# MirceaKitsune/python_raytracer

Measured on AMD Instinct MI355X. Metric: Mrays/s (primary+bounce), higher is better.
Workload: dtype f64; 1 GPU; mods/default 3840x2160 spp8 max_bounces8 (BASELINE config 3/4); width=3840, height=2160, samples=8, primary_rays=62725130, bounce_rays=75192856, partition=(x ^ y) % 1, traversed=True, fast_draws=32, frames_in_flight=1, scene_flow=pre-selected camera chunks (fixture), rng_retraced_rays=0, rng_table=static seeds: draw table + ray table built once before the timed region, reused

## Files before the change

### python_raytracer_amd/csrc/vrt_kernels.hip

```cpp
#include <hip/hip_runtime.h>
#include <stdint.h>
#include <stdio.h>
#include <stdlib.h>
#include <string.h>

#include <atomic>
#include <mutex>
#include <vector>

#include "../../include/vrt.h"
#include "vrt_math.h"

#pragma clang fp contract(off)

#define VRT_WAVE 64
#define VRT_BLOCK 256

static thread_local int g_last_hip_error = 0;
#define HIP_TRY(expr)                                   \
    do {                                                \
        hipError_t e__ = (expr);                        \
        if (e__ != hipSuccess) {                        \
            g_last_hip_error = (int)e__;                \
            return VRT_ERR_HIP;                         \
// ... 8 lines not shown
struct ProfScope {
    hipStream_t s;
    bool on;
    ProfEvent e;
    ProfScope(hipStream_t stream, int kind) : s(stream), on(g_prof_on && ((g_prof_kinds >> kind) & 1u)) {
        if (!on) return;
        e.kind = kind;
        if (hipEventCreate(&e.a) != hipSuccess) { on = false; return; }
        if (hipEventCreate(&e.b) != hipSuccess) { (void)hipEventDestroy(e.a); on = false; return; }
        (void)hipEventRecord(e.a, s);
    }
    ~ProfScope() {
        if (!on) return;
        (void)hipEventRecord(e.b, s);
        std::lock_guard<std::mutex> lock(g_prof_mu);
        g_prof.push_back(e);
    }
};

__host__ __device__ static inline int64_t voxel_offset(int cs, int lx, int ly, int lz) {
    int nb = cs >> 3;
    int brick = (((lx >> 3) * nb) + (ly >> 3)) * nb + (lz >> 3);
    int micro = ((((lx >> 2) & 1) * 2) + ((ly >> 2) & 1)) * 2 + ((lz >> 2) & 1);
    int vox = (((lx & 3) * 4) + (ly & 3)) * 4 + (lz & 3);
    return (int64_t)brick * 512 + micro * 64 + vox;
}

template <class ST>
__host__ __device__ static inline void pixel_setup(const ST& st, int x, int y, double& dir_x, double& dir_y,
                                                   double& detail, int& n) {
    dir_x = -1 + ((double)x / (double)st.width) * 2;
    dir_y = -1 + ((double)y / (double)st.height) * 2;
    detail = 1 - __builtin_fabs(dir_x * dir_y) * st.lod_edge;
    double r = __builtin_rint((double)st.samples * detail);
    n = r > 1 ? (int)r : 1;
}

struct TileGeom {
    const int32_t* pixels;
    int64_t n_px;
    int32_t smax;
};

template <class ST>
__host__ __device__ static inline uint64_t ray_seed(const ST& st, int smax, int x, int y, int s) {
    if (st.seed_nonce == 0) return (uint64_t)((uint32_t)(1 + x) * (uint32_t)(1 + y) * (uint32_t)(1 + s));
    return ((uint64_t)y * (uint64_t)st.width + (uint64_t)x) * (uint64_t)smax + (uint64_t)s + st.seed_nonce;
}

#define VRT_PLAN_MAGIC 0x5652544e414c5032ull
struct PlanHeader {
    uint64_t magic, n_px, n_slots, n_distinct, settings_hash, n_words;
    uint64_t full_frame;
    uint64_t pad;
};
static_assert(sizeof(PlanHeader) == 64, "plan header is 64 bytes");

static uint64_t plan_hash(const vrt_settings* st, int64_t n_px) {
    uint64_t h = 0xcbf29ce484222325ull;
    auto mix = [&](uint64_t v) { h = (h ^ v) * 0x100000001b3ull; };
    union { double d; uint64_t u; } c;
    c.d = st->lod_edge;
    mix((uint64_t)st->width);
    mix((uint64_t)st->height);
    mix((uint64_t)st->samples);
    mix(c.u);
    mix((uint64_t)n_px);
    return h;
}

#define VRT_SCAN_WORDS 1024

__global__ void __launch_bounds__(VRT_BLOCK) plan_mark_kernel(vrt_settings st, TileGeom g, uint32_t* bitmap, PlanHeader* hdr) {
    int64_t p = (int64_t)blockIdx.x * VRT_BLOCK + threadIdx.x;
    if (p >= g.n_px) return;
    int x = g.pixels[2 * p], y = g.pixels[2 * p + 1];
    if ((int64_t)x * st.height + y != p) hdr->full_frame = 0;
    double dx, dy, det;
    int ns;
    pixel_setup(st, x, y, dx, dy, det, ns);
    const uint32_t base = (uint32_t)(1 + x) * (uint32_t)(1 + y);
    for (int s = 0; s < ns; s++) {
        const uint32_t seed = base * (uint32_t)(1 + s);
        const uint32_t bit = 1u << (seed & 31);
        if (!(bitmap[seed >> 5] & bit)) atomicOr(&bitmap[seed >> 5], bit);
    }
}

__global__ void __launch_bounds__(VRT_BLOCK) plan_blocksum_kernel(const uint32_t* bitmap, int64_t n_words,
                                                                   uint32_t* block_sums) {
    __shared__ uint32_t s_sum[VRT_BLOCK / VRT_WAVE];
    int64_t w0 = (int64_t)blockIdx.x * VRT_SCAN_WORDS + threadIdx.x * 4;
    uint32_t c = 0;
    for (int k = 0; k < 4; k++)
        if (w0 + k < n_words) c += __popc(bitmap[w0 + k]);
    for (int o = 32; o > 0; o >>= 1) c += __shfl_down(c, o);
    if ((threadIdx.x & 63) == 0) s_sum[threadIdx.x >> 6] = c;
    __syncthreads();
    if (threadIdx.x == 0) block_sums[blockIdx.x] = s_sum[0] + s_sum[1] + s_sum[2] + s_sum[3];
}

__global__ void __launch_bounds__(VRT_BLOCK) plan_scan_sums_kernel(uint32_t* block_sums, int64_t n_blocks,
                                                                    PlanHeader* hdr) {
    __shared__ uint32_t s_part[VRT_BLOCK];
    __shared__ uint32_t s_carry;
    if (threadIdx.x == 0) s_carry = 0;
    __syncthreads();
    for (int64_t base = 0; base < n_blocks; base += VRT_BLOCK) {
        int64_t i = base + threadIdx.x;
        uint32_t v = i < n_blocks ? block_sums[i] : 0;
        s_part[threadIdx.x] = v;
        __syncthreads();
        for (int o = 1; o < VRT_BLOCK; o <<= 1) {
            uint32_t t = threadIdx.x >= (unsigned)o ? s_part[threadIdx.x - o] : 0;
            __syncthreads();
            s_part[threadIdx.x] += t;
            __syncthreads();
        }
        uint32_t incl = s_part[threadIdx.x];
        uint32_t carry = s_carry;
        if (i < n_blocks) block_sums[i] = carry + incl - v;
        __syncthreads();
        if (threadIdx.x == VRT_BLOCK - 1) s_carry = carry + incl;
        __syncthreads();
    }
    if (threadIdx.x == 0) hdr->n_distinct = s_carry;
}

__global__ void __launch_bounds__(VRT_BLOCK) plan_compact_kernel(const uint32_t* bitmap, int64_t n_words,
                                                                  const uint32_t* block_sums, uint32_t* prefix,
                                                                  uint32_t* seed_list) {
    __shared__ uint32_t s_part[VRT_BLOCK];
    int64_t w0 = (int64_t)blockIdx.x * VRT_SCAN_WORDS + threadIdx.x * 4;
    uint32_t words[4], c = 0;
    for (int k = 0; k < 4; k++) {
        words[k] = (w0 + k < n_words) ? bitmap[w0 + k] : 0;
        c += __popc(words[k]);
    }
    s_part[threadIdx.x] = c;
    __syncthreads();
    for (int o = 1; o < VRT_BLOCK; o <<= 1) {
        uint32_t t = threadIdx.x >= (unsigned)o ? s_part[threadIdx.x - o] : 0;
        __syncthreads();
        s_part[threadIdx.x] += t;
        __syncthreads();
    }
    uint32_t pos = block_sums[blockIdx.x] + s_part[threadIdx.x] - c;
    for (int k = 0; k < 4; k++) {
        if (w0 + k >= n_words) break;
        prefix[w0 + k] = pos;
        uint32_t w = words[k];
        while (w) {
            int b = __ffs(w) - 1;
            w &= w - 1;
            seed_list[pos++] = (uint32_t)((w0 + k) * 32 + b);
        }
    }
}

__global__ void __launch_bounds__(VRT_BLOCK) plan_index_kernel(vrt_settings st, TileGeom g, const uint32_t* bitmap,
                                                                const uint32_t* prefix, uint32_t* ray_seedidx) {
    int64_t i = (int64_t)blockIdx.x * VRT_BLOCK + threadIdx.x;
    if (i >= g.n_px * g.smax) return;
    int64_t p = i / g.smax;
    int s = (int)(i - p * g.smax);
    int x = g.pixels[2 * p], y = g.pixels[2 * p + 1];
    double dx, dy, det;
    int ns;
    pixel_setup(st, x, y, dx, dy, det, ns);
    uint32_t out = 0xffffffffu;
    if (s < ns) {
        const uint32_t seed = (uint32_t)(1 + x) * (uint32_t)(1 + y) * (uint32_t)(1 + s);
        const uint32_t w = bitmap[seed >> 5];
        out = prefix[seed >> 5] + __popc(w & ((1u << (seed & 31)) - 1u));
    }
    ray_seedidx[i] = out;
}

struct MtInit { uint32_t v[624]; };
static constexpr MtInit make_mt_init() {
    MtInit t{};
    t.v[0] = 19650218u;
    for (int i = 1; i < 624; i++) t.v[i] = 1812433253u * (t.v[i - 1] ^ (t.v[i - 1] >> 30)) + (uint32_t)i;
    return t;
}
__constant__ MtInit c_mt_init = make_mt_init();

__device__ __forceinline__ uint32_t mt_temper(uint32_t y) {
    y ^= (y >> 11);
    y ^= (y << 7) & 0x9d2c5680u;
    y ^= (y << 15) & 0xefc60000u;
    y ^= (y >> 18);
    return y;
}
__device__ __forceinline__ uint32_t mt_out(uint32_t sk, uint32_t sk1, uint32_t sk397) {
    uint32_t y = (sk & 0x80000000u) | (sk1 & 0x7fffffffu);
    uint32_t v = sk397 ^ (y >> 1) ^ ((y & 1u) ? 0x9908b0dfu : 0u);
    return mt_temper(v);
}
__device__ __forceinline__ double mt_res53(uint32_t a, uint32_t b) {
    return ((double)(a >> 5) * 67108864.0 + (double)(b >> 6)) * (1.0 / 9007199254740992.0);
}

template <bool PAIR>
__device__ __forceinline__ void mt_seed_draws(uint64_t seed, int D, double* out) {
    const int K = 2 * D;
    const uint32_t key0 = (uint32_t)seed, key1 = (uint32_t)(seed >> 32);
    const uint32_t addA = key0;
    const uint32_t addB = key1 ? key1 + 1u : key0;
    const uint32_t* init = c_mt_init.v;
    uint32_t m = init[0];
    m = (init[1] ^ ((m ^ (m >> 30)) * 1664525u)) + addA;
    const uint32_t first1 = m;
#pragma unroll 2
    for (int i = 2; i < 624; i++) m = (init[i] ^ ((m ^ (m >> 30)) * 1664525u)) + (((i - 1) & 1) ? addB : addA);
    const uint32_t mt1 = (first1 ^ ((m ^ (m >> 30)) * 1664525u)) + ((623 & 1) ? addB : addA);
#define VRT_MT_STEP(p, q, i)                                                            \
    p = (init[i] ^ ((p ^ (p >> 30)) * 1664525u)) + ((((i) - 1) & 1) ? addB : addA);      \
    q = (p ^ ((q ^ (q >> 30)) * 1566083941u)) - (uint32_t)(i);
    uint32_t p = first1, q = mt1;
#pragma unroll 2
    for (int i = 2; i < 397; i++) { VRT_MT_STEP(p, q, i) }
    uint32_t rp = first1, rq = mt1;
    uint32_t s397, s398, s2;
    { VRT_MT_STEP(p, q, 397) }
    s397 = q;
    { VRT_MT_STEP(p, q, 398) }
    s398 = q;
    { VRT_MT_STEP(rp, rq, 2) }
// ... 409 lines not shown
    const uint32_t* list;
    const uint32_t* list_count;
    const double* draws;
    int32_t n_draws, draw_stride;
    int32_t first_draw;
    int32_t per_pixel;
    double lens;
    int32_t t_hit, t_end;
    int32_t max_iters;
    int32_t chunk;
    int32_t brick_lds_off;
    int32_t pool_lds_off;
    int32_t pool_swap_min;
    int32_t pool_refill_min;
    int32_t pool_keep;
    int32_t list_seed;
    union {
        int32_t prefix_draws;
        int32_t slot_stride;
        int32_t max_hits;
    };
    int32_t ct_cells;
    int32_t ct_identity;
    int32_t trav_words;
    int32_t snap_flags;
    int32_t bm_window;
    int32_t wt_on;
    int32_t wt_lds_off;
    int32_t wt_cells[3];
    int32_t wt_min[3];
    int32_t wt_words;
    const uint32_t* wt_table;
    uint32_t* ray_rgba;
    union {
        vrt_ray* rays;
        vrt_hit* hits;
        vrt_cast_ray* out_rays;
    };
    uint64_t* stats;
    uint32_t* retrace_list;
    union {
        uint32_t* retrace_count;
        int32_t* path_counts;
    };
    unsigned long long* pow_global;
    unsigned long long* queue_head;
    const PlanHeader* plan_hdr;
    uint32_t* tile_heads;
    int32_t tile_px_log2;
    int32_t tile_log2;
    int32_t tile_ntx, tile_nty;
    uint32_t retrace_cap;
    uint32_t list_cap;
};
#define VRT_VIEW_WORDS 10
#define VRT_VIEWS_LDS_MAX 96

__device__ __noinline__ int3 snap_generic3(int res, int imx, int imy, int imz, int lx, int ly, int lz) {
    int3 o;
    o.x = (int)__builtin_floor((double)(lx + imx) / (double)res) * res - imx;
    o.y = (int)__builtin_floor((double)(ly + imy) / (double)res) * res - imy;
    o.z = (int)__builtin_floor((double)(lz + imz) / (double)res) * res - imz;
    return o;
}

template <class PT>
__device__ __forceinline__ uint32_t chunk_entry_i(const PT& P, const __attribute__((address_space(3))) uint32_t* ct, int cx, int cy,
                                                  int cz, int d0, int d1, int d2, bool lds, bool identity) {
    if ((unsigned)cx >= (unsigned)d0 || (unsigned)cy >= (unsigned)d1 || (unsigned)cz >= (unsigned)d2) return 0;
    const int i = (cx * d1 + cy) * d2 + cz;
    if (lds) return ct[i];
    if (identity) return (uint32_t)(i + 1) | (1u << 24);
    uint32_t e = P.chunk_table[i];
    asm volatile("" : "+v"(e));
    return e;
}
__device__ __forceinline__ const uint8_t* chunk_base(const MarchParams& P, uint32_t entry) {
    return P.voxels + ((int64_t)((entry & 0xffffffu) - 1u) << (3 * P.cs_shift));
}

__device__ __forceinline__ int trav_cell(bool has_keys, int ccx, int ccy, int ccz, int to0, int to1, int to2, int td0, int td1,
                                         int td2) {
    if (!has_keys) return -1;
    const int cx = ccx - to0;
    const int cy = ccy - to1;
    const int cz = ccz - to2;
    if ((unsigned)cx >= (unsigned)td0 || (unsigned)cy >= (unsigned)td1 || (unsigned)cz >= (unsigned)td2) return -2;
    return (cx * td1 + cy) * td2 + cz;
}

struct PowCache {
    unsigned long long* keys;
    unsigned long long* vals;
    unsigned long long* gkeys;
    unsigned long long* gvals;
};
__device__ __forceinline__ unsigned pow_hash(unsigned long long bits) {
    unsigned h = (unsigned)(bits >> 32) * 0x9e3779b1u + (unsigned)bits * 0x85ebca6bu;
    return h >> 24;
}
#define VRT_PW_PROBES 4
#ifndef VRT_POW_INLINE
#define VRT_POW_INLINE __noinline__
#endif
__device__ VRT_POW_INLINE double pow_miss(unsigned long long* keys, unsigned long long* vals, unsigned long long* gkeys,
                                        unsigned long long* gvals, double x, double y) {
// ... 88 lines not shown
    double d0, d1, d2;
    uint32_t view;
};

__device__ __forceinline__ unsigned long long wave_first_u64(unsigned long long v) {
    const unsigned lo = __builtin_amdgcn_readfirstlane((unsigned)v), hi = __builtin_amdgcn_readfirstlane((unsigned)(v >> 32));
    return ((unsigned long long)hi << 32) | lo;
}

enum { LANE_IDLE = 0, LANE_MARCH = 1, LANE_HIT = 2, LANE_ENDED = 3, LANE_ENDED_BROKE = 4, LANE_ENDED_EXHAUSTED = 5 };
__device__ __forceinline__ int opaque_zero() {
    int z = 0;
    asm volatile("" : "+v"(z));
    return z;
}
enum { COLD_POS = 0, COLD_ROT = 3, COLD_DIST_MIN = 7, COLD_POW_Y, COLD_LOD_BOUNCES, COLD_MAX_LIGHT, COLD_MAX_BOUNCES1,
       COLD_SHUTTER, COLD_CS, COLD_INV_CS, COLD_N };
enum { C_LOOKUP = 0, C_NBR, C_CGET, C_HIT, C_ADV, C_NLOCAL };

typedef __attribute__((address_space(3))) uint32_t lds_u32;
typedef __attribute__((address_space(3))) double lds_f64;
typedef __attribute__((address_space(3))) unsigned long long lds_u64;
typedef __attribute__((address_space(3))) char lds_char;

struct MarchCtx {
    const lds_char* tab;
    int tl[3];
    const lds_u32* ct;
    lds_u32* bm;
    const lds_f64* mats;
    const lds_f64* cold;
    lds_u32* tot;
    PowCache pc;
    __amdgpu_buffer_rsrc_t vox;
    unsigned cs4;
    double cs, inv_cs;
    bool kept_cs;
    bool has_bm, tile;

    int td[3];
    int toc[3], oc[3], dm[3];
    const lds_char* wt;
    int wb[3];
    unsigned cs3;
    const lds_char* vw;
};
#define COLD(i) C.cold[(i) + opaque_zero()]
enum { CF_HAS_BM = 1, CF_CT_LDS = 2, CF_CT_IDENTITY = 4, CF_HAS_KEYS = 8, CF_BM_WINDOW = 16 };

#ifdef VRT_DIAG
enum { DG_PASSES = 0, DG_CYC_REFILL, DG_CYC_MARCH, DG_CYC_HIT, DG_CYC_END, DG_ITERS, DG_MARCH_LANES, DG_HIT_EXEC,
       DG_HIT_LANES, DG_END_EXEC, DG_END_LANES, DG_REFILL_EXEC, DG_REFILL_LANES, DG_WAVE_CYCLES, DG_SNAP_ITERS,
       DG_SNAP_LANES, DG_BRICK_VISITS, DG_SWAPS, DG_SWAP_LANES, DG_EVICT_LANES, DG_CYC_SWAP, DG_VOID_LANES,
#ifdef VRT_DIAG_HIST
       DG_NV1, DG_H1 = DG_NV1 + 8, DG_N = DG_H1 + 8
#else
       DG_N
#endif
};
__device__ unsigned long long g_diag[DG_N];
__device__ unsigned long long g_diag_t[5];
#define DG_ADD(idx_, val_)                                                                                      \
    do {                                                                                                        \
        const unsigned long long v_ = (unsigned long long)(val_);   \
        const unsigned long long e_ = __ballot(1);                                                              \
        if ((int)(threadIdx.x & 63) == __ffsll((long long)e_) - 1) dg.acc[idx_] += v_;                           \
    } while (0)
#define DG_TIME() __builtin_amdgcn_s_memtime()
struct DgLane {
    __attribute__((address_space(3))) unsigned long long* acc;
    unsigned brick;
    unsigned long long bv;
};
#define DG_BRICK()                                                                                                     \
    do {                                                                                                               \
        const unsigned key_ = (((unsigned)(int)__builtin_floor(r.px) >> 3) & 1023u) |                                  \
                              ((((unsigned)(int)__builtin_floor(r.py) >> 3) & 1023u) << 10) |                          \
                              ((((unsigned)(int)__builtin_floor(r.pz) >> 3) & 1023u) << 20);                           \
        dg.bv += key_ != dg.brick ? 1 : 0;                                                                             \
        dg.brick = key_;                                                                                               \
    } while (0)
#else
struct DgLane {};
#define DG_ADD(i, v)
#define DG_BRICK()
#endif
#ifdef VRT_ISA_MARK
#define VRT_MARK(name) asm volatile("; @@" name)
#else
#define VRT_MARK(name)
#endif

__device__ __forceinline__ void floor3_i32(double x, double y, double z, int& fx, int& fy, int& fz) {
    double a, b, c;
    const double magic = 6755399441055744.0;
    asm volatile(
        "s_setreg_imm32_b32 hwreg(HW_REG_MODE, 2, 2), 2\n\t"
        "v_add_f64 %0, %3, %6\n\t"
        "v_add_f64 %1, %4, %6\n\t"
        "v_add_f64 %2, %5, %6\n\t"
        "s_setreg_imm32_b32 hwreg(HW_REG_MODE, 2, 2), 0"
        : "=&v"(a), "=&v"(b), "=&v"(c)
        : "v"(x), "v"(y), "v"(z), "s"(magic));
    fx = __double2loint(a);
    fy = __double2loint(b);
    fz = __double2loint(c);
// ... 1986 lines not shown
        if (tile_ticket(Q, (uint32_t)(ts & 7) * per_head + k, first)) {
            first_ray = first;
            break;
        }
    }
    return ts;
}
#define VRT_POOL_STATE_WORD (13 * 2 * VRT_POOL_SLOTS + 9 * VRT_POOL_SLOTS)
#define VRT_POOL_OFF_WORD (13 * 2 * VRT_POOL_SLOTS + 7 * VRT_POOL_SLOTS)

template <int SPEC, int RESMODE, int PERPIX = 0, bool W = false, bool DEFER = false, bool TILE = false>
__global__ void __launch_bounds__(VRT_BLOCK, VRT_WAVES_PER_SIMD) march_pool_kernel(MarchParams P) {
    static_assert(!TILE || DEFER, "tiled hand-out: the instances for scenes beyond the caches");
    static_assert(!W || (RESMODE != 2 && SPEC == 8), "march_step_w");
    static_assert(!(W && DEFER), "deferred key comparison: the shipped march step");
    __shared__ MarchSharedT<W> S;
    extern __shared__ __align__(16) unsigned char s_dyn[];
    MarchCtx C;
    march_prologue<W>(P, S, s_dyn, C);
    const int wave_in_block = threadIdx.x >> 6;
    const int lane = threadIdx.x & 63;
    lds_u64* const pool = (lds_u64*)(s_dyn + P.pool_lds_off + wave_in_block * VRT_POOL_WAVE_BYTES);
    lds_u32* const pool_state = (lds_u32*)pool + VRT_POOL_STATE_WORD;
    if (lane < VRT_POOL_SLOTS) pool_state[lane] = (uint32_t)LANE_IDLE;
    __syncthreads();

    const int64_t count = P.n;
    const int64_t chunk = P.chunk > 0 ? P.chunk : VRT_CHUNK;
    const int64_t tail_start = count - (int64_t)gridDim.x * (2 * VRT_BLOCK);
    int64_t next = 0, range_end = 0;
    bool more = true;
    bool tiled = false;
    int ts = 0;
    if constexpr (TILE) {
        tiled = P.tile_heads != nullptr && P.plan_hdr->full_frame != 0;
        unsigned xcc = 0;
        xcc = __builtin_amdgcn_s_getreg((3 << 11) | 20);
        ts = (int)(xcc & 7u);
    }

    Ray r;
    ray_clear(r);
    int state = LANE_IDLE;
    SeenList<false> sl = seen_unused();
    LkState lk = lk_unused();
    uint64_t wmin_key = 0;
    DG_LANE(dg);
#ifdef VRT_DIAG
    const unsigned long long dg_t_start = __builtin_amdgcn_s_memrealtime();
    unsigned long long dg_t_empty = 0;
    const unsigned long long dg_start = DG_TIME();
#endif

    auto refill = [&]() {
        unsigned long long idle_mask = __ballot(state == LANE_IDLE);
#ifdef VRT_DIAG
        DG_ADD(DG_REFILL_EXEC, 1);
        DG_ADD(DG_REFILL_LANES, __popcll(idle_mask));
#endif
        while (idle_mask != 0ull && (next < range_end || more)) {
            if (TILE && next >= range_end && tiled) {
                int64_t first = -1;
                ts = tile_take(P, ts, lane, chunk, first);
                if (first < 0) {
                    more = false;
#ifdef VRT_DIAG
                    if (!dg_t_empty) dg_t_empty = __builtin_amdgcn_s_memrealtime();
#endif
                    break;
                }
                next = first;
                range_end = first + chunk;
            } else if (next >= range_end) {
                unsigned long long base = 0;
                if (lane == 0) base = atomicAdd(P.queue_head, (unsigned long long)chunk);
                base = wave_first_u64(base);
                if ((int64_t)base >= count) {
                    more = false;
#ifdef VRT_DIAG
                    if (!dg_t_empty) dg_t_empty = __builtin_amdgcn_s_memrealtime();
#endif
                    break;
                }
                next = (int64_t)base;
                range_end = next + chunk < count ? next + chunk : count;
            }
            const unsigned rank = __builtin_amdgcn_mbcnt_hi((unsigned)(idle_mask >> 32),
                                                            __builtin_amdgcn_mbcnt_lo((unsigned)idle_mask, 0u));
            const int64_t k = next + rank;
            next += __popcll(idle_mask);
            if (state == LANE_IDLE && k < range_end) {
                SeenList<false> none;
                none.n = 0;
                if (take_ray<false, false, PERPIX, W>(P, C, k, r, dg, W ? wmin_key : 0ull, none)) state = LANE_MARCH;
            }
            idle_mask = __ballot(state == LANE_IDLE);
        }
    };
    constexpr bool PASS_COUNTS = W || VRT_PASS_COUNTS;
    int32_t tot[C_NLOCAL];
#pragma unroll
    for (int j = 0; j < C_NLOCAL; j++) tot[j] = 0;
    constexpr bool FUSE_ENDED = (VRT_POOL_FUSE & 1) != 0, FUSE_HIT = (VRT_POOL_FUSE & 2) != 0;
    unsigned pass = 0;
    int stalled = 0;
    for (;; pass++) {
#ifdef VRT_DIAG
        DG_ADD(DG_PASSES, 1);
#endif
        VRT_MARK("pass");
        if (PASS_COUNTS) {
#pragma unroll
            for (int j = 0; j < C_NLOCAL; j++) tot[j] = 0;
        }
        const int sstate = lane < VRT_POOL_SLOTS ? (int)__hip_atomic_load(pool_state + lane, __ATOMIC_RELAXED, __HIP_MEMORY_SCOPE_WAVEFRONT) : -1;
        const bool lane_i = state == LANE_IDLE;
        const unsigned long long l_m = __ballot(state == LANE_MARCH), l_h = __ballot(state == LANE_HIT),
                                 l_e = __ballot(state >= LANE_ENDED), l_i = __ballot(lane_i);
        const unsigned long long s_m = __ballot(sstate == LANE_MARCH), s_h = __ballot(sstate == LANE_HIT),
                                 s_e = __ballot(sstate >= LANE_ENDED), s_f = __ballot(sstate == LANE_IDLE);
        const int n_m = (int)(__popcll(l_m) + __popcll(s_m)), n_h = (int)(__popcll(l_h) + __popcll(s_h)),
                  n_e = (int)(__popcll(l_e) + __popcll(s_e));
        const bool rays_left = next < range_end || more;
        if (stalled > 4096) {
            if (lane == 0) atomicAdd(&S.stats[VRT_S_STALLED], 1ull);
            break;
        }
        const bool evict_ok = rays_left && ((TILE && tiled) ? !(ts & 0x80) : range_end < tail_start);
        const bool can_add = rays_left && (l_i != 0ull || (evict_ok && s_f != 0ull));
        int target;
        if (rays_left) {
            if (n_h >= P.t_hit) target = LANE_HIT;
            else if (n_e >= P.t_end) target = LANE_ENDED;
            else if (n_m > 0 || can_add) target = LANE_MARCH;
            else target = n_h >= n_e ? LANE_HIT : LANE_ENDED;
        } else {
            if (n_m + n_h + n_e == 0) break;
            target = LANE_MARCH;
        }
        const bool tail = !rays_left;
        if (C.has_bm && (pass & 7u) == 0u && (!rays_left || next < range_end)) {
            if (lane == 0) S.wtmp[wave_in_block] = rays_left ? (uint32_t)(P.ray0 + next) : 0xffffffffu;
            if (!lane_i) atomicMin(&S.wtmp[wave_in_block], (uint32_t)(P.ray0 + r.off));
            if (sstate > LANE_IDLE)
                atomicMin(&S.wtmp[wave_in_block],
                          (uint32_t)(P.ray0 + __hip_atomic_load((lds_u32*)pool + VRT_POOL_OFF_WORD + lane, __ATOMIC_RELAXED, __HIP_MEMORY_SCOPE_WAVEFRONT)));
            wmin_key = publish_wave_min(S, wave_in_block, S.wtmp[wave_in_block]);
        }
// ... 556 lines not shown

static constexpr int D_SLOW = 113;
static constexpr int64_t SLOW_CAP_MIN = 1 << 18;
static constexpr int64_t SLOW_CAP_MAX = 1 << 22;
static constexpr int64_t FULL_CAP = 1 << 12;

static int env_int(const char* name, int dflt) {
    const char* e = getenv(name);
    return e ? atoi(e) : dflt;
}

static int64_t batch_rays() {
    static int64_t b = 0;
    if (!b) {
        int l = env_int("VRT_BATCH_LOG2", 28);
        if (l < 12) l = 12;
        if (l > 30) l = 30;
        b = (int64_t)1 << l;
    }
    return b;
}

static inline int grid_for(int64_t n) { return (int)((n + VRT_BLOCK - 1) / VRT_BLOCK); }

__global__ void __launch_bounds__(VRT_BLOCK) clear_words_kernel(uint32_t* p, int n) {
    for (int i = blockIdx.x * VRT_BLOCK + threadIdx.x; i < n; i += gridDim.x * VRT_BLOCK) p[i] = 0u;
}
static inline void clear_words(void* p, int64_t bytes, hipStream_t stream) {
    hipLaunchKernelGGL(clear_words_kernel, dim3(1), dim3(VRT_BLOCK), 0, stream, (uint32_t*)p, (int)(bytes / 4));
}
__global__ void __launch_bounds__(VRT_BLOCK) frame_begin_kernel(uint32_t* stats, int n_stats, uint32_t* count, int n_count, uint32_t* pow_memo,
                                                                int n_pow, unsigned long long* keys, int64_t n_keys) {
    const int64_t t = (int64_t)blockIdx.x * VRT_BLOCK + threadIdx.x, step = (int64_t)gridDim.x * VRT_BLOCK;
    for (int64_t i = t; i < n_keys; i += step) keys[i] = ~0ull;
    if (blockIdx.x != 0) return;
    for (int i = threadIdx.x; i < n_stats; i += VRT_BLOCK) stats[i] = 0u;
    for (int i = threadIdx.x; i < n_count; i += VRT_BLOCK) count[i] = 0u;
    for (int i = threadIdx.x; i < n_pow; i += VRT_BLOCK) pow_memo[i] = 0u;
}
static inline void frame_begin(uint64_t* d_stats, void* count, int n_count_words, void* pow_memo, int n_pow_words, uint64_t* keys, int64_t n_keys,
                               hipStream_t stream) {
    const int64_t kb = (n_keys + VRT_BLOCK * 8 - 1) / (VRT_BLOCK * 8);
    hipLaunchKernelGGL(frame_begin_kernel, dim3((unsigned)(kb < 1 ? 1 : (kb > 1024 ? 1024 : kb))), dim3(VRT_BLOCK), 0, stream, (uint32_t*)d_stats,
                       (int)(2 * VRT_NSTATS), (uint32_t*)count, n_count_words, (uint32_t*)pow_memo, n_pow_words, (unsigned long long*)keys, n_keys);
}
static inline void frame_begin(uint64_t* d_stats, void* count, int n_count_words, void* pow_memo, int n_pow_words, const vrt_traversed* trav,
                               hipStream_t stream) {
    const bool reset = trav && trav->d_keys && trav->reset;
    frame_begin(d_stats, count, n_count_words, pow_memo, n_pow_words, reset ? trav->d_keys : nullptr,
                reset ? (int64_t)trav->dims[0] * trav->dims[1] * trav->dims[2] : 0, stream);
}
static inline int64_t align256(int64_t v) { return (v + 255) & ~(int64_t)255; }
static inline const uint32_t* plan_seedidx(const void* d_plan, int64_t slots) { return (const uint32_t*)((const char*)d_plan + 64 + align256(slots * 4)); }

static int march_grid(int64_t n) {
    static int cap = -1;
    if (cap < 0) {
        cap = env_int("VRT_MARCH_GRID", 256 * VRT_WAVES_PER_SIMD);
        if (cap < 1) cap = 1;
    }
    int64_t g = (n + VRT_BLOCK * 4 - 1) / (VRT_BLOCK * 4);
    if (g < 1) g = 1;
    return (int)(g < cap ? g : cap);
}

struct PowMemo {
    int dev;
    double y;
    unsigned long long* buf;
};
static constexpr int MAX_MEMOS = 64;
static std::mutex g_memo_mu;
static PowMemo g_memos[MAX_MEMOS];
static int g_n_memos = 0;
static bool memo_per_frame() {
    static int per_frame = -1;
    if (per_frame < 0) {
        const char* e = getenv("VRT_POW_MEMO");
        per_frame = (e && e[0] == 'f') ? 1 : 0;
    }
    return per_frame != 0;
}
static unsigned long long* device_pow_memo(double y) {
    if (memo_per_frame()) return nullptr;
    int dev = 0;
    if (hipGetDevice(&dev) != hipSuccess) return nullptr;
    std::lock_guard<std::mutex> lock(g_memo_mu);
    for (int i = 0; i < g_n_memos; i++)
        if (g_memos[i].dev == dev && g_memos[i].y == y) return g_memos[i].buf;
    return nullptr;
}
struct FrameMemo { unsigned long long* p; int clear; };
static FrameMemo frame_memo(const vrt_settings* st, void* in_workspace, bool any_rays) {
    unsigned long long* m = device_pow_memo(1 + st->falloff);
    return {m ? m : (unsigned long long*)in_workspace, !m && any_rays ? 4 * VRT_PW_SLOTS : 0};
}

static int march_chunk(int64_t n) {
    static int c = -2;
    if (c == -2) {
        const char* e = getenv("VRT_CHUNK");
        c = e ? atoi(e) : -1;
        if (e && c < 0) c = 0;
    }
    if (c >= 0) return c;
    return n <= ((int64_t)1 << 22) ? 128 : (n <= ((int64_t)1 << 24) ? 256 : VRT_CHUNK);
// ... 121 lines not shown
}

int vrt_world_tables_bytes(const int32_t* dims, int32_t cs, int64_t* bytes) {
    if (!dims || !bytes || cs < 8 || (cs & (cs - 1)) || cs > 256) return VRT_ERR_ARG;
    const int64_t w = world_table_words(dims, cs);
    if (w < 0) return VRT_ERR_ARG;
    *bytes = w * 4;
    return VRT_OK;
}

int vrt_world_tables_build(const int32_t* dims, int32_t cs, uint32_t* d_tables, int64_t bytes, void* stream_) {
    hipStream_t stream = (hipStream_t)stream_;
    int64_t need = 0;
    int rc = vrt_world_tables_bytes(dims, cs, &need);
    if (rc != VRT_OK) return rc;
    if (need == 0 || !d_tables) return VRT_ERR_ARG;
    if (bytes < need) return VRT_ERR_WORKSPACE;
    int shift = 0;
    while ((1 << shift) < cs) shift++;
    hipLaunchKernelGGL(world_tables_kernel, dim3((unsigned)grid_for(need / 4)), dim3(VRT_BLOCK), 0, stream, (int)dims[0], (int)dims[1],
                       (int)dims[2], (int)cs, shift, d_tables);
    HIP_TRY(hipGetLastError());
    return VRT_OK;
}

int vrt_occupancy_build(const uint8_t* d_voxels, int64_t n_bytes, uint64_t* d_occupancy, void* stream_) {
    hipStream_t stream = (hipStream_t)stream_;
    if (n_bytes < 0 || (n_bytes & 63) || (n_bytes > 0 && (!d_voxels || !d_occupancy))) return VRT_ERR_ARG;
    if (n_bytes == 0) return VRT_OK;
    const int64_t words = n_bytes / 64;
    if (words * 4 > (int64_t)0x7fffffff * VRT_BLOCK) return VRT_ERR_ARG;
    hipLaunchKernelGGL(occupancy_kernel, dim3((unsigned)grid_for(words * 4)), dim3(VRT_BLOCK), 0, stream, d_voxels, words,
                       d_occupancy);
    HIP_TRY(hipGetLastError());
    return VRT_OK;
}

static int64_t plan_words(const vrt_settings* st) {
    int64_t max_seed = (int64_t)st->width * st->height * vrt_max_samples(st);
    return max_seed / 32 + 1;
}
static int plan_supported(const vrt_settings* st) {
    double m = (double)st->width * (double)st->height * (double)vrt_max_samples(st);
    return m < 4294967296.0;
}

int vrt_plan_bytes(const vrt_settings* st, int64_t n_px, int64_t* plan_bytes, int64_t* scratch_bytes) {
    if (check_settings(st) != VRT_OK || n_px < 0 || !plan_bytes || !scratch_bytes) return VRT_ERR_ARG;
    if (!plan_supported(st)) return VRT_ERR_ARG;
    int64_t slots = n_px * vrt_max_samples(st);
    if (slots >= 4294967295ll) return VRT_ERR_ARG;
    int64_t words = plan_words(st);
    int64_t blocks = (words + VRT_SCAN_WORDS - 1) / VRT_SCAN_WORDS;
    *plan_bytes = 64 + align256(slots * 4) + align256(slots * 4) + 256;
    *scratch_bytes = align256(words * 4) + align256(words * 4) + align256(blocks * 4) + 256;
    return VRT_OK;
}

int vrt_plan_build(const vrt_settings* st, const int32_t* d_pixels_xy, int64_t n_px, void* d_plan, int64_t plan_bytes,
                   void* d_scratch, int64_t scratch_bytes, void* stream_) {
    hipStream_t stream = (hipStream_t)stream_;
    int64_t need_plan = 0, need_scratch = 0;
    int rc = vrt_plan_bytes(st, n_px, &need_plan, &need_scratch);
    if (rc != VRT_OK) return rc;
    if (!d_plan || !d_scratch || (n_px > 0 && !d_pixels_xy)) return VRT_ERR_ARG;
    if (plan_bytes < need_plan || scratch_bytes < need_scratch) return VRT_ERR_WORKSPACE;
    const int smax = vrt_max_samples(st);
    const int64_t slots = n_px * smax;
    const int64_t words = plan_words(st);
    const int64_t blocks = (words + VRT_SCAN_WORDS - 1) / VRT_SCAN_WORDS;
    char* pl = (char*)d_plan;
    PlanHeader* hdr = (PlanHeader*)pl;
    uint32_t* seed_list = (uint32_t*)(pl + 64);
    uint32_t* ray_seedidx = (uint32_t*)(pl + 64 + align256(slots * 4));
    char* sc = (char*)d_scratch;
    uint32_t* bitmap = (uint32_t*)sc;
    uint32_t* prefix = (uint32_t*)(sc + align256(words * 4));
    uint32_t* block_sums = (uint32_t*)(sc + 2 * align256(words * 4));
    PlanHeader h;
    h.magic = VRT_PLAN_MAGIC;
    h.n_px = (uint64_t)n_px;
    h.n_slots = (uint64_t)slots;
    h.n_distinct = 0;
    h.settings_hash = plan_hash(st, n_px);
    h.n_words = (uint64_t)words;
    h.full_frame = n_px == (int64_t)st->width * st->height ? 1 : 0;
    h.pad = 0;
    HIP_TRY(hipMemcpyAsync(hdr, &h, sizeof h, hipMemcpyHostToDevice, stream));
    HIP_TRY(hipMemsetAsync(bitmap, 0, (size_t)words * 4, stream));
    const TileGeom g = {d_pixels_xy, n_px, smax};
    if (n_px > 0) hipLaunchKernelGGL(plan_mark_kernel, dim3(grid_for(n_px)), dim3(VRT_BLOCK), 0, stream, *st, g, bitmap, hdr);
    hipLaunchKernelGGL(plan_blocksum_kernel, dim3((unsigned)blocks), dim3(VRT_BLOCK), 0, stream, bitmap, words, block_sums);
    hipLaunchKernelGGL(plan_scan_sums_kernel, dim3(1), dim3(VRT_BLOCK), 0, stream, block_sums, blocks, hdr);
    hipLaunchKernelGGL(plan_compact_kernel, dim3((unsigned)blocks), dim3(VRT_BLOCK), 0, stream, bitmap, words, block_sums,
                       prefix, seed_list);
    if (slots > 0)
        hipLaunchKernelGGL(plan_index_kernel, dim3(grid_for(slots)), dim3(VRT_BLOCK), 0, stream, *st, g, bitmap, prefix,
                           ray_seedidx);
    HIP_TRY(hipGetLastError());
    return VRT_OK;
}

struct WsLayout {
    int64_t rays;
    int64_t batch;
    int64_t slow_cap;
    int64_t full_cap;
    int64_t off_table, off_slow, off_full, off_tab, off_rgba, off_list, off_list_full, off_count, off_pow, total;
};
static WsLayout ws_layout(const vrt_settings* st, int64_t n_px, int64_t n_distinct, int fast_draws, int external) {
    WsLayout w;
    w.rays = n_px * vrt_max_samples(st);
    w.batch = w.rays < batch_rays() ? w.rays : batch_rays();
    if (w.batch < 1) w.batch = 1;
    int64_t o = 0;
    auto take = [&](int64_t bytes) { int64_t r = o; o += align256(bytes); return r; };
    w.off_table = take((external & VRT_WS_DRAW_TABLE) ? 0 : (n_distinct > 0 ? n_distinct : 1) * (int64_t)fast_draws * 8);
    w.slow_cap = w.batch / 64;
    if (w.slow_cap < SLOW_CAP_MIN) w.slow_cap = w.batch < SLOW_CAP_MIN ? w.batch : SLOW_CAP_MIN;
    if (w.slow_cap > SLOW_CAP_MAX) w.slow_cap = SLOW_CAP_MAX;
    w.off_slow = take(w.slow_cap * VRT_SLOW_STRIDE * 8);
    w.full_cap = w.slow_cap < FULL_CAP ? w.slow_cap : FULL_CAP;
    w.off_full = take(w.full_cap * D_FULL_DEV * 8);
    const int64_t tab_records = ray_table_per_pixel(*st) ? n_px : w.rays;
    w.off_tab = take((external & VRT_WS_RAY_TABLE) ? 0 : (tab_records > 0 ? tab_records : 1) * 8 * VRT_RAY_WORDS);
    w.off_rgba = take(w.rays * 4);
    w.off_list = take(w.slow_cap * 4);
    w.off_list_full = take(w.full_cap * 4);
    w.off_count = take(256 + 8 * 128);
    w.off_pow = take(2 * VRT_PW_SLOTS * 8);
    w.total = o;
    return w;
}

static int fast_draws_ok(int32_t d) { return d == 32 || d == 64; }

int vrt_workspace_bytes(const vrt_settings* st, int64_t n_px, int64_t n_distinct, int32_t fast_draws, int32_t external,
                        int64_t* bytes) {
    if (check_settings(st) != VRT_OK || n_px < 0 || n_distinct < 0 || !bytes || !fast_draws_ok(fast_draws)) return VRT_ERR_ARG;
    if (external & ~(VRT_WS_DRAW_TABLE | VRT_WS_RAY_TABLE)) return VRT_ERR_ARG;
    *bytes = ws_layout(st, n_px, n_distinct, fast_draws, external).total;
    return VRT_OK;
}

static inline bool within(double v, double lim) { return __builtin_fabs(v) <= lim; }

static int fill_scene_params(MarchParams& P, const vrt_scene* sc, const vrt_settings* st, const vrt_camera* cam,
                             const vrt_traversed* trav, uint64_t* d_stats) {
    if (!sc || check_settings(st) != VRT_OK) return VRT_ERR_ARG;
    if (sc->chunk_size != st->chunk_size || sc->n_materials < 0 || sc->n_materials > 255) return VRT_ERR_ARG;
    if (!sc->d_chunk_table || (sc->n_slots > 0 && !sc->d_voxels) || (sc->n_materials > 0 && !sc->d_materials))
// ... 64 lines not shown
        for (int a = 0; a < 3; a++) {
            if (trav->dims[a] <= 0 || (trav->origin[a] % st->chunk_size) != 0) return VRT_ERR_ARG;
            if (trav->origin[a] < -(1ll << 28) || trav->origin[a] + (int64_t)trav->dims[a] * st->chunk_size > (1ll << 28)) return VRT_ERR_ARG;
            P.t_origin_c[a] = (int32_t)(trav->origin[a] / st->chunk_size);
            P.t_dims[a] = trav->dims[a];
            tcells *= trav->dims[a];
        }
        if (tcells >= (1ll << 31)) return VRT_ERR_ARG;
        P.t_keys = trav->d_keys;
        const int trav_lds = env_int("VRT_TRAV_LDS", 1);
        const int64_t words = (tcells + 31) / 32;
        int64_t wt_bytes = 0;
        if (P.wt_on)
            for (int a = 0; a < 3; a++) wt_bytes += ((int64_t)P.wt_cells[a] + 2 * VRT_WT_GUARD) * 4;
        const int64_t room = 160 * 1024 / VRT_WAVES_PER_SIMD - 2 * 1024 -
                             (int64_t)(P.wt_on ? sizeof(MarchSharedT<true>) : sizeof(MarchShared)) -
                             (int64_t)sc->n_materials * 64 - (int64_t)P.ct_cells * 4 - wt_bytes - 64;
        P.bm_window = -1;
        const int win_env = env_int("VRT_TRAV_WINDOW", 1);
        if (trav_lds && win_env != 2 && tcells <= VRT_TRAV_LDS_MAX && words * 4 <= room) {
            P.trav_words = (int32_t)words;
        } else if (cam && trav_lds && win_env != 0 && 32 * 32 * 32 / 8 <= room && trav->dims[0] >= 32 && trav->dims[1] >= 32 &&
                   trav->dims[2] >= 32 && trav->dims[0] < 1024 + 32 && trav->dims[1] < 1024 + 32 && trav->dims[2] < 1024 + 32) {
            int w = 0;
            for (int a = 0; a < 3; a++) {
                const double p = cam->pos[a];
                int64_t c = (int64_t)__builtin_floor(p / st->chunk_size) - P.t_origin_c[a] - 16;
                c = c < 0 ? 0 : (c > trav->dims[a] - 32 ? trav->dims[a] - 32 : c);
                w |= (int)c << (10 * a);
            }
            P.bm_window = w;
            P.trav_words = 32 * 32 * 32 / 32;
        }
    }
    P.stats = d_stats;
    P.g.pixels = nullptr;
    P.g.n_px = 0;
    P.g.smax = 1;
    P.ray_seedidx = nullptr;
    P.expl_detail = nullptr;
    P.list = nullptr;
    P.list_count = nullptr;
    P.ray_rgba = nullptr;
    P.rays = nullptr;
    P.retrace_list = nullptr;
    P.retrace_count = nullptr;
    P.pow_global = nullptr;
    P.queue_head = nullptr;
    P.plan_hdr = nullptr;
    P.tile_heads = nullptr;
    P.tile_px_log2 = P.tile_log2 = P.tile_ntx = P.tile_nty = 0;
    P.retrace_cap = 0;
    P.list_cap = 0;
    P.chunk = march_chunk(0);
    P.first_draw = 0;
    P.brick_lds_off = 0;
    P.pool_lds_off = 0;
    P.pool_swap_min = 1;
    P.pool_refill_min = 1;
    P.pool_keep = 64;
    P.prefix_draws = 0;
    P.list_seed = 0;
    P.per_pixel = 0;
    P.lens = 0.0;
    march_policy(march_big_scene(sc), 0, P.t_hit, P.t_end, P.max_iters);
    return VRT_OK;
}
static int fill_params(MarchParams& P, const vrt_scene* sc, const vrt_settings* st, const vrt_camera* cam,
                       const vrt_traversed* trav, uint64_t* d_stats) {
    if (!cam) return VRT_ERR_ARG;
    return fill_scene_params(P, sc, st, cam, trav, d_stats);
}

}

static int lookup_mode() {
    static int m = -1;
    if (m < 0) {
        m = env_int("VRT_LOOKUP", 0);
        if (m < 0 || m > 2) m = 0;
    }
    return m;
}
#ifndef VRT_POOL_DEFAULT
#define VRT_POOL_DEFAULT 1
#endif
static bool march_pool() { return env_int("VRT_POOL", VRT_POOL_DEFAULT) != 0; }
static void pool_policy(MarchParams& P, bool big_scene) {
    static int h = -2, e, sw, rf, kp, it;
    if (h == -2) {
        h = env_int("VRT_POOL_T_HIT", -1);
        e = env_int("VRT_POOL_T_END", -1);
        sw = env_int("VRT_POOL_SWAP_MIN", -1);
        rf = env_int("VRT_POOL_REFILL_MIN", -1);
        kp = env_int("VRT_POOL_KEEP", -1);
        it = env_int("VRT_POOL_ITERS", -1);
    }
    const int cap = 64 + VRT_POOL_SLOTS;
    auto pick = [](int env, int dflt, int lo, int hi) { const int v = env >= 0 ? env : dflt; return v < lo ? lo : (v > hi ? hi : v); };
    P.t_hit = pick(h, big_scene ? 48 : 40, 1, cap);
    P.t_end = pick(e, big_scene ? 32 : 60, 1, cap);
    P.pool_swap_min = pick(sw, big_scene ? 4 : 8, 1, 64);
    P.pool_refill_min = pick(rf, 8, 1, 64);
    P.pool_keep = pick(kp, 40, 1, 64);
    P.max_iters = pick(it, big_scene ? 5 : 3, 1, 64);
}
// ... 484 lines not shown
    if (st->seed_nonce && n_distinct != rays) return VRT_ERR_ARG;
    WsLayout w = ws_layout(st, n_px, n_distinct, fast_draws,
                           (d_draw_table ? VRT_WS_DRAW_TABLE : 0) | (d_ray_table ? VRT_WS_RAY_TABLE : 0));
    if (workspace_bytes < w.total) return VRT_ERR_WORKSPACE;
    char* ws = (char*)d_workspace;
    const double* table = d_draw_table ? d_draw_table : (const double*)(ws + w.off_table);
    double* t_slow = (double*)(ws + w.off_slow);
    uint32_t* rgba = d_ray_rgba ? d_ray_rgba : (uint32_t*)(ws + w.off_rgba);
    uint32_t* list = (uint32_t*)(ws + w.off_list);
    uint32_t* count = (uint32_t*)(ws + w.off_count);
    const FrameMemo memo = frame_memo(st, ws + w.off_pow, n_px > 0);
    frame_begin(d_stats, count, n_px > 0 ? 64 + 8 * 32 : 0, memo.p, memo.clear, trav, stream);
    if (n_px == 0) return VRT_OK;
    const TileGeom g = {d_pixels_xy, n_px, smax};
    if (!d_draw_table) {
        ProfScope ps(stream, VRT_PROF_RNG);
        rc = seed_draw_table(st, g, d_plan, n_distinct, fast_draws, (double*)(ws + w.off_table), stream);
        if (rc != VRT_OK) return rc;
    }
    RayTab tab = ray_tab_at(d_ray_table ? const_cast<double*>(d_ray_table) : (double*)(ws + w.off_tab), rays);
    const int resmode = res_mode(scene);
    const bool deep = march_deep(scene, resmode);
    const bool big_scene = march_big_scene(scene);
    int per_pixel = ray_table_per_pixel(*st) ? 1 : 0;
    if (!d_ray_table && !per_pixel && !d_rays && !P.wt_on && march_eight(resmode, deep, lookup_mode()) && env_int("VRT_FUSE_RAYGEN", 1) != 0)
        per_pixel = 2;
    if (!d_ray_table && per_pixel != 2) {
        ProfScope ps(stream, VRT_PROF_RAYGEN);
        hipLaunchKernelGGL(raygen_tile_kernel, dim3(grid_for(per_pixel ? n_px : rays)), dim3(VRT_BLOCK), 0, stream, *st, cam->lens,
                           g, ray_seedidx, table, (int)fast_draws, tab, per_pixel);
    }
    P.g = g;
    P.ray_seedidx = st->seed_nonce ? nullptr : ray_seedidx;
    P.ray_rgba = rgba;
    P.rays = d_rays;
    P.pow_global = memo.p;
    P.first_draw = 1 + (st->dof != 0.0 ? 2 : 0);
    P.per_pixel = per_pixel;
    P.lens = cam->lens;
    P.tab = tab;
    const MarchTiers tiers = {table, fast_draws, t_slow, (double*)(ws + w.off_full), list, (uint32_t*)(ws + w.off_list_full), count,
                              w.slow_cap, w.full_cap};
    for (int64_t ray0 = 0; ray0 < rays; ray0 += w.batch) {
        const int64_t n = (rays - ray0) < w.batch ? (rays - ray0) : w.batch;
        if (ray0 != 0) clear_words(count, 256 + 8 * 128, stream);
        P.ray0 = ray0;
        P.n = n;
        P.chunk = march_chunk(n);
        march_policy(big_scene, n, P.t_hit, P.t_end, P.max_iters);
        set_tier(P, tiers, 0);
        MarchParams F = P;
        F.wt_on = !d_rays && march_wt_ok(P, resmode, deep);
        const bool pool = !d_rays && pool_plan(F);
        const int tile_env = env_int("VRT_TILED", 0);
        if (pool && (big_scene || tile_env == 2) && F.trav_words == 0 && ray0 == 0 && n == rays && n_px == (int64_t)st->width * st->height &&
            F.chunk > 0 && F.chunk % smax == 0 && st->height % (F.chunk / smax) == 0 && tile_env != 0) {
            const int px = F.chunk / smax;
            const int ntx = (st->width + px - 1) / px, nty = st->height / px;
            int lg = 1, lpx = 0;
            while ((1 << lg) < ntx || (1 << lg) < nty) lg++;
            while ((1 << lpx) < px) lpx++;
            if ((1 << lpx) == px && lpx + 2 * lg <= 31 && lpx + 2 * lg >= 3) {
                F.plan_hdr = (const PlanHeader*)d_plan;
                F.tile_heads = count + 64;
                F.tile_px_log2 = lpx;
                F.tile_log2 = lg;
                F.tile_ntx = ntx;
                F.tile_nty = nty;
            }
        }
        {
            ProfScope ps(stream, VRT_PROF_MARCH);
            rc = launch_march(F, march_grid(n), resmode, deep, pool, d_rays != nullptr, false, stream);
            if (rc != VRT_OK) return rc;
        }
        ProfScope ps(stream, VRT_PROF_RETRACE);
        set_tier(P, tiers, 1);
        P.prefix_draws = pool ? fast_draws : 0;
        launch_march(P, 256, resmode, deep, false, d_rays != nullptr, true, stream);
        P.prefix_draws = 0;
        set_tier(P, tiers, 2);
        launch_march(P, 64, resmode, deep, false, d_rays != nullptr, true, stream);
    }
    if (d_rgba_f32 || d_image_u8) {
        ProfScope ps(stream, VRT_PROF_RESOLVE);
        hipLaunchKernelGGL(resolve_kernel, dim3(resolve_grid(st, n_px)), dim3(VRT_BLOCK), 0, stream, *st, g, (const PlanHeader*)d_plan, rgba,
                           d_rgba_f32, d_image_u8);
    }
    HIP_TRY(hipGetLastError());
    return VRT_OK;
}

int vrt_views_workspace_bytes(const vrt_settings* st, int32_t n_views, int64_t n_px, int64_t* bytes) {
    if (check_settings(st) != VRT_OK || n_views < 1 || n_px < 0 || !bytes) return VRT_ERR_ARG;
    if ((int64_t)n_views * n_px * vrt_max_samples(st) >= 4294967295ll) return VRT_ERR_ARG;
    *bytes = views_layout(st, n_views, n_px).total;
    return VRT_OK;
}

int vrt_render_views(const vrt_scene* scene, const vrt_settings* st, const vrt_camera* d_cams, int32_t n_views,
                     const int32_t* d_pixels_xy, int64_t n_px, const void* d_plan, int64_t n_distinct, int32_t fast_draws,
                     const double* d_draw_table, const double* d_ray_table, void* d_workspace, int64_t workspace_bytes,
                     float* d_rgba_f32, uint8_t* d_image_u8, uint32_t* d_ray_rgba, vrt_ray* d_rays, uint64_t* d_stats,
                     const vrt_traversed* traversed, void* stream_) {
    hipStream_t stream = (hipStream_t)stream_;
    if (!d_cams || n_views < 1) return VRT_ERR_ARG;
// ... 896 lines not shown
```

Before: 29950 Mrays/s.

## Skip unused sample slots in refill using a precomputed per-ray used mask

The plan index kernel now writes a bitmask marking which per-pixel sample slots are real (s < ns) and counts the unused ones in the plan header. In the masked per-pixel path, the march kernel's refill reads this mask and compacts only used slots onto idle lanes with permute, zeroing the RGBA of skipped slots. This avoids spending refill trips and take_ray calls on slots that would exit immediately. In exchange the refill loop gets more complex, and the plan grows by one bit per slot.

```diff
diff --git a/python_raytracer_amd/csrc/vrt_kernels.hip b/python_raytracer_amd/csrc/vrt_kernels.hip
--- a/python_raytracer_amd/csrc/vrt_kernels.hip
+++ b/python_raytracer_amd/csrc/vrt_kernels.hip
@@ -84,7 +84,7 @@
 struct PlanHeader {
     uint64_t magic, n_px, n_slots, n_distinct, settings_hash, n_words;
     uint64_t full_frame;
-    uint64_t pad;
+    uint64_t n_unused;
 };
 static_assert(sizeof(PlanHeader) == 64, "plan header is 64 bytes");
 
@@ -191,7 +191,8 @@
 }
 
 __global__ void __launch_bounds__(VRT_BLOCK) plan_index_kernel(vrt_settings st, TileGeom g, const uint32_t* bitmap,
-                                                                const uint32_t* prefix, uint32_t* ray_seedidx) {
+                                                                const uint32_t* prefix, uint32_t* ray_seedidx,
+                                                                unsigned long long* used_mask, PlanHeader* hdr) {
     int64_t i = (int64_t)blockIdx.x * VRT_BLOCK + threadIdx.x;
     if (i >= g.n_px * g.smax) return;
     int64_t p = i / g.smax;
@@ -207,6 +208,11 @@
         out = prefix[seed >> 5] + __popc(w & ((1u << (seed & 31)) - 1u));
     }
     ray_seedidx[i] = out;
+    const unsigned long long used = __ballot(s < ns), unused = __ballot(s >= ns);
+    if ((threadIdx.x & 63) == 0) {
+        used_mask[i >> 6] = used;
+        if (unused != 0ull) atomicAdd((unsigned long long*)&hdr->n_unused, (unsigned long long)__popcll(unused));
+    }
 }
 
 struct MtInit { uint32_t v[624]; };
@@ -722,6 +728,7 @@
     int32_t tile_ntx, tile_nty;
     uint32_t retrace_cap;
     uint32_t list_cap;
+    const unsigned long long* used_mask;
 };
 #define VRT_VIEW_WORDS 10
 #define VRT_VIEWS_LDS_MAX 96
@@ -916,6 +923,7 @@
 enum { DG_PASSES = 0, DG_CYC_REFILL, DG_CYC_MARCH, DG_CYC_HIT, DG_CYC_END, DG_ITERS, DG_MARCH_LANES, DG_HIT_EXEC,
        DG_HIT_LANES, DG_END_EXEC, DG_END_LANES, DG_REFILL_EXEC, DG_REFILL_LANES, DG_WAVE_CYCLES, DG_SNAP_ITERS,
        DG_SNAP_LANES, DG_BRICK_VISITS, DG_SWAPS, DG_SWAP_LANES, DG_EVICT_LANES, DG_CYC_SWAP, DG_VOID_LANES,
+       DG_REFILL_TRIPS, DG_REFILL_TRIP_LANES, DG_REFILL_UNUSED_MET,
 #ifdef VRT_DIAG_HIST
        DG_NV1, DG_H1 = DG_NV1 + 8, DG_N = DG_H1 + 8
 #else
@@ -3008,48 +3016,126 @@
     const unsigned long long dg_start = DG_TIME();
 #endif
 
+    constexpr bool MASKED = PERPIX == 3 && !TILE;
     auto refill = [&]() {
         unsigned long long idle_mask = __ballot(state == LANE_IDLE);
 #ifdef VRT_DIAG
         DG_ADD(DG_REFILL_EXEC, 1);
         DG_ADD(DG_REFILL_LANES, __popcll(idle_mask));
 #endif
+        if constexpr (!MASKED) {
+            while (idle_mask != 0ull && (next < range_end || more)) {
+                if (TILE && next >= range_end && tiled) {
+                    int64_t first = -1;
+                    ts = tile_take(P, ts, lane, chunk, first);
+                    if (first < 0) {
+                        more = false;
+#ifdef VRT_DIAG
+                        if (!dg_t_empty) dg_t_empty = __builtin_amdgcn_s_memrealtime();
+#endif
+                        break;
+                    }
+                    next = first;
+                    range_end = first + chunk;
+                } else if (next >= range_end) {
+                    unsigned long long base = 0;
+                    if (lane == 0) base = atomicAdd(P.queue_head, (unsigned long long)chunk);
+                    base = wave_first_u64(base);
+                    if ((int64_t)base >= count) {
+                        more = false;
+#ifdef VRT_DIAG
+                        if (!dg_t_empty) dg_t_empty = __builtin_amdgcn_s_memrealtime();
+#endif
+                        break;
+                    }
+                    next = (int64_t)base;
+                    range_end = next + chunk < count ? next + chunk : count;
+                }
+                const unsigned rank = __builtin_amdgcn_mbcnt_hi((unsigned)(idle_mask >> 32),
+                                                                __builtin_amdgcn_mbcnt_lo((unsigned)idle_mask, 0u));
+                const int64_t k = next + rank;
+                next += __popcll(idle_mask);
+#ifdef VRT_DIAG
+                if (__ballot(state == LANE_IDLE && k < range_end) != 0ull) { DG_ADD(DG_REFILL_TRIPS, 1); DG_ADD(DG_REFILL_TRIP_LANES, __popcll(__ballot(state == LANE_IDLE && k < range_end))); }
+#endif
+                if (state == LANE_IDLE && k < range_end) {
+                    SeenList<false> none;
+                    none.n = 0;
+                    if (take_ray<false, false, PERPIX, W>(P, C, k, r, dg, W ? wmin_key : 0ull, none)) state = LANE_MARCH;
+                }
+                idle_mask = __ballot(state == LANE_IDLE);
+            }
+            return;
+        }
         while (idle_mask != 0ull && (next < range_end || more)) {
-            if (TILE && next >= range_end && tiled) {
-                int64_t first = -1;
-                ts = tile_take(P, ts, lane, chunk, first);
-                if (first < 0) {
-                    more = false;
-#ifdef VRT_DIAG
-                    if (!dg_t_empty) dg_t_empty = __builtin_amdgcn_s_memrealtime();
-#endif
-                    break;
-                }
-                next = first;
-                range_end = first + chunk;
-            } else if (next >= range_end) {
-                unsigned long long base = 0;
-                if (lane == 0) base = atomicAdd(P.queue_head, (unsigned long long)chunk);
-                base = wave_first_u64(base);
-                if ((int64_t)base >= count) {
-                    more = false;
-#ifdef VRT_DIAG
-                    if (!dg_t_empty) dg_t_empty = __builtin_amdgcn_s_memrealtime();
-#endif
-                    break;
-                }
-                next = (int64_t)base;
-                range_end = next + chunk < count ? next + chunk : count;
-            }
             const unsigned rank = __builtin_amdgcn_mbcnt_hi((unsigned)(idle_mask >> 32),
                                                             __builtin_amdgcn_mbcnt_lo((unsigned)idle_mask, 0u));
-            const int64_t k = next + rank;
-            next += __popcll(idle_mask);
-            if (state == LANE_IDLE && k < range_end) {
+            const int n_idle = (int)__popcll(idle_mask);
+            int64_t k = 0;
+            bool has = false;
+            int done = 0;
+            const unsigned long long* const um = fresh_args(P).used_mask;
+            do {
+                if (next >= range_end) {
+                    unsigned long long base = 0;
+                    if (lane == 0) base = atomicAdd(P.queue_head, (unsigned long long)chunk);
+                    base = wave_first_u64(base);
+                    if ((int64_t)base >= count) {
+                        more = false;
+#ifdef VRT_DIAG
+                        if (!dg_t_empty) dg_t_empty = __builtin_amdgcn_s_memrealtime();
+#endif
+                        break;
+                    }
+                    next = (int64_t)base;
+                    range_end = next + chunk < count ? next + chunk : count;
+                }
+                if (um != nullptr) {
+                    const auto& Q = fresh_args(P);
+                    const uint64_t s0 = (uint64_t)(Q.ray0 + next);
+                    const auto* mw = (const __attribute__((address_space(4))) unsigned long long*)um + (s0 >> 6);
+                    const unsigned sh = (unsigned)s0 & 63u;
+                    unsigned long long win = (mw[0] >> sh) | ((mw[1] << 1) << (63u - sh));
+                    const int64_t left = range_end - next;
+                    const int span = left < 64 ? (int)left : 64;
+                    if (span < 64) win &= (1ull << span) - 1ull;
+                    const int want = n_idle - done, n_used = (int)__popcll(win);
+                    const int urank = (int)__builtin_amdgcn_mbcnt_hi((unsigned)(win >> 32), __builtin_amdgcn_mbcnt_lo((unsigned)win, 0u));
+                    const bool ubit = ((win >> lane) & 1ull) != 0ull;
+                    int adv = span;
+                    if (n_used > want) adv = __ffsll((long long)__ballot(ubit && urank == want - 1));
+                    const int slot_of_rank = __builtin_amdgcn_ds_permute((ubit ? urank : 63) << 2, lane);
+                    const int j = (int)rank - done;
+                    const int src = __builtin_amdgcn_ds_bpermute((j & 63) << 2, slot_of_rank);
+                    const bool got = j >= 0 && j < n_used;
+                    k = got ? next + src : k;
+                    has = has | got;
+                    if (!ubit && lane < adv && Q.ray_rgba) Q.ray_rgba[Q.ray0 + next + lane] = 0;
+                    next += adv;
+                    done += n_used < want ? n_used : want;
+                } else {
+                    k = next + rank;
+                    has = k < range_end;
+                    next += n_idle;
+                    done = n_idle;
+                }
+            } while (done < n_idle && (next < range_end || more));
+            const bool mine = (state == LANE_IDLE) & has;
+#ifdef VRT_DIAG
+            bool dg_met = false;
+            if (__ballot(mine) != 0ull) { DG_ADD(DG_REFILL_TRIPS, 1); DG_ADD(DG_REFILL_TRIP_LANES, __popcll(__ballot(mine))); }
+#endif
+            if (mine) {
                 SeenList<false> none;
                 none.n = 0;
                 if (take_ray<false, false, PERPIX, W>(P, C, k, r, dg, W ? wmin_key : 0ull, none)) state = LANE_MARCH;
+#ifdef VRT_DIAG
+                else dg_met = true;
+#endif
             }
+#ifdef VRT_DIAG
+            if (um != nullptr) DG_ADD(DG_REFILL_UNUSED_MET, __popcll(__ballot(dg_met)));
+#endif
             idle_mask = __ballot(state == LANE_IDLE);
         }
     };
@@ -3712,6 +3798,10 @@
 }
 static inline int64_t align256(int64_t v) { return (v + 255) & ~(int64_t)255; }
 static inline const uint32_t* plan_seedidx(const void* d_plan, int64_t slots) { return (const uint32_t*)((const char*)d_plan + 64 + align256(slots * 4)); }
+static inline int64_t plan_mask_bytes(int64_t slots) { return align256(8 * ((slots + 63) / 64)); }
+static inline const unsigned long long* plan_used_mask(const void* d_plan, int64_t slots) {
+    return (const unsigned long long*)((const char*)d_plan + 64 + 2 * align256(slots * 4));
+}
 
 static int march_grid(int64_t n) {
     static int cap = -1;
@@ -3939,7 +4029,7 @@
     if (slots >= 4294967295ll) return VRT_ERR_ARG;
     int64_t words = plan_words(st);
     int64_t blocks = (words + VRT_SCAN_WORDS - 1) / VRT_SCAN_WORDS;
-    *plan_bytes = 64 + align256(slots * 4) + align256(slots * 4) + 256;
+    *plan_bytes = 64 + align256(slots * 4) + align256(slots * 4) + plan_mask_bytes(slots) + 256;
     *scratch_bytes = align256(words * 4) + align256(words * 4) + align256(blocks * 4) + 256;
     return VRT_OK;
 }
@@ -3972,7 +4062,7 @@
     h.settings_hash = plan_hash(st, n_px);
     h.n_words = (uint64_t)words;
     h.full_frame = n_px == (int64_t)st->width * st->height ? 1 : 0;
-    h.pad = 0;
+    h.n_unused = 0;
     HIP_TRY(hipMemcpyAsync(hdr, &h, sizeof h, hipMemcpyHostToDevice, stream));
     HIP_TRY(hipMemsetAsync(bitmap, 0, (size_t)words * 4, stream));
     const TileGeom g = {d_pixels_xy, n_px, smax};
@@ -3983,7 +4073,7 @@
                        prefix, seed_list);
     if (slots > 0)
         hipLaunchKernelGGL(plan_index_kernel, dim3(grid_for(slots)), dim3(VRT_BLOCK), 0, stream, *st, g, bitmap, prefix,
-                           ray_seedidx);
+                           ray_seedidx, const_cast<unsigned long long*>(plan_used_mask(d_plan, slots)), hdr);
     HIP_TRY(hipGetLastError());
     return VRT_OK;
 }
@@ -4154,6 +4244,7 @@
     P.tile_px_log2 = P.tile_log2 = P.tile_ntx = P.tile_nty = 0;
     P.retrace_cap = 0;
     P.list_cap = 0;
+    P.used_mask = nullptr;
     P.chunk = march_chunk(0);
     P.first_draw = 0;
     P.brick_lds_off = 0;
@@ -4744,6 +4835,7 @@
         MarchParams F = P;
         F.wt_on = !d_rays && march_wt_ok(P, resmode, deep);
         const bool pool = !d_rays && pool_plan(F);
+        if (pool && F.per_pixel == 2 && st->lod_edge != 0.0 && env_int("VRT_USED_MASK", 1) != 0) F.used_mask = plan_used_mask(d_plan, rays);
         const int tile_env = env_int("VRT_TILED", 0);
         if (pool && (big_scene || tile_env == 2) && F.trav_words == 0 && ray0 == 0 && n == rays && n_px == (int64_t)st->width * st->height &&
             F.chunk > 0 && F.chunk % smax == 0 && st->height % (F.chunk / smax) == 0 && tile_env != 0) {
```

After: 29490 Mrays/s. -1.5%, worse.
